# dotchen/LAV

Hardware: NVIDIA H100
Metric: agent_frames_per_s (higher is better)
Workload: dtype fp16 storage, fp32 accumulate (wgmma f16 / mma.sync f16; saturating stores)

## Files before the change

### include/lav_b200.h

```cpp
#ifndef LAV_B200_H
#define LAV_B200_H

#include <stddef.h>
#include <stdint.h>

#ifdef __cplusplus
extern "C" {
#endif

#define LAVB_ABI_VERSION 3

int lavb_abi_version(void);
const char* lavb_last_error(void);
int lavb_device_cc(void);

enum { LAVB_F32 = 0, LAVB_BF16 = 1, LAVB_F16 = 2 };
int lavb_h16_dtype(void);

int lavb_paint(const float* d_pts, int n, int pt_stride,
               const float* d_sem, int ncam, int c_in, int h, int w,
               long long s_cam, long long s_c, long long s_y, long long s_x,
               const float* h_cams, int mode,
               float* d_out, int out_stride, int out_col0, int copy_cols, void* stream);

// ... 180 lines not shown
size_t lavb_det_peaks_workspace_bytes(int batch, int ncls);
int lavb_det_peaks(const float* d_center, const float* d_box, const float* d_ori, int batch, int h, int w, int ncls,
                   float min_score, int max_det, float* d_packed, void* d_workspace, void* stream);

int lavb_crop_bilinear(const void* d_feat, int dtype, int b, int h, int w, int c, const int* d_frame_idx,
                       const float* d_theta, int k, int crop, void* d_out, void* stream);
int lavb_crop_bilinear_u8(const uint8_t* d_map, int b, int c, int h, int w, const int* d_frame_idx, const float* d_theta,
                          int k, int crop, float* d_out, void* stream);
int lavb_crop_bilinear_bwd(const float* d_gout, int b, int h, int w, int c, const int* d_frame_idx, const float* d_theta,
                           int k, int crop, float* d_gfeat, void* stream);

int lavb_convert(const void* d_src, int src_dtype, void* d_dst, int dst_dtype, long long count, void* stream);

int lavb_conv_umma(const lavb_conv_desc* h_desc, void* stream);

int lavb_conv7x7s2_umma(const void* d_in, int n, int h, int w, int cin, const void* d_w, const float* d_bias, void* d_out,
                        void* stream);

int lavb_conv3x3_umma(const void* d_in, int n, int h, int w, int cin, int stride, const void* d_w, int cout, const float* d_bias,
                      const float* d_scale, const float* d_shift, int pre_relu, void* d_out, void* stream);

typedef struct lavb_conv_pair_desc {
  const void* in; void* out; const void* res;
  int n, h, w, c, dil, post_relu;
  const void* w1; const float* bias1;
  const void* w2; const float* shift2;
} lavb_conv_pair_desc;
int lavb_conv_pair_umma(const lavb_conv_pair_desc* h_desc, void* stream);
int lavb_conv_pair_set_trace(void* d_buf, int tiles_per_cta);

// ... 15 lines not shown
```

### lav_b200/capi.py

```python
import ctypes as C
import os

_HERE = os.path.dirname(os.path.abspath(__file__))
LIB_PATH = os.path.join(_HERE, "_lib", "liblavb200.so")

F32, BF16, F16 = 0, 1, 2


class LavbError(RuntimeError):
    pass


class ConvDesc(C.Structure):
    _fields_ = [
        ("inp", C.c_void_p), ("in_dtype", C.c_int), ("n", C.c_int), ("hin", C.c_int), ("win", C.c_int), ("cin", C.c_int),
        ("in_cstride", C.c_int), ("in_coff", C.c_int),
        ("out", C.c_void_p), ("out_dtype", C.c_int), ("hout", C.c_int), ("wout", C.c_int), ("cout", C.c_int),
        ("out_cstride", C.c_int), ("out_coff", C.c_int),
        ("hog", C.c_int), ("wog", C.c_int),
        ("in_sy", C.c_int), ("in_sx", C.c_int), ("out_sy", C.c_int), ("out_sx", C.c_int), ("out_oy", C.c_int), ("out_ox", C.c_int),
        ("ntaps", C.c_int), ("dy", C.c_int * 16), ("dx", C.c_int * 16),
        ("w", C.c_void_p), ("bias", C.c_void_p), ("scale", C.c_void_p), ("shift", C.c_void_p),
        ("res", C.c_void_p), ("res_dtype", C.c_int), ("res_cstride", C.c_int), ("res_coff", C.c_int),
        ("pre_relu", C.c_int), ("post_relu", C.c_int), ("sigmoid", C.c_int), ("d2s_nout", C.c_int),
    ]


class ConvPairDesc(C.Structure):
    _fields_ = [
        ("inp", C.c_void_p), ("out", C.c_void_p), ("res", C.c_void_p),
        ("n", C.c_int), ("h", C.c_int), ("w", C.c_int), ("c", C.c_int), ("dil", C.c_int), ("post_relu", C.c_int),
        ("w1", C.c_void_p), ("bias1", C.c_void_p),
        ("w2", C.c_void_p), ("shift2", C.c_void_p),
    ]


class ControlConfig(C.Structure):
    _fields_ = [
        ("aim_point", C.c_int * 8), ("speed_ratio", C.c_double * 8),
# ... 103 lines not shown
    "lavb_det_peaks_workspace_bytes": (C.c_size_t, [C.c_int, C.c_int]),
    "lavb_det_peaks": (C.c_int, [C.c_void_p, C.c_void_p, C.c_void_p, C.c_int, C.c_int, C.c_int, C.c_int, C.c_float, C.c_int,
                                 C.c_void_p, C.c_void_p, C.c_void_p]),
    "lavb_crop_bilinear": (C.c_int, [C.c_void_p, C.c_int, C.c_int, C.c_int, C.c_int, C.c_int, C.c_void_p, C.c_void_p, C.c_int,
                                     C.c_int, C.c_void_p, C.c_void_p]),
    "lavb_crop_bilinear_u8": (C.c_int, [C.c_void_p, C.c_int, C.c_int, C.c_int, C.c_int, C.c_void_p, C.c_void_p, C.c_int, C.c_int,
                                        C.c_void_p, C.c_void_p]),
    "lavb_cast_gru": (C.c_int, [C.c_void_p, C.c_int, C.c_void_p, C.c_void_p, C.c_void_p, C.c_void_p, C.c_void_p, C.c_void_p, C.c_int,
                                C.c_int, C.c_void_p, C.c_void_p]),
    "lavb_conv_pair_set_trace": (C.c_int, [C.c_void_p, C.c_int]),
    "lavb_crop_bilinear_bwd": (C.c_int, [C.c_void_p, C.c_int, C.c_int, C.c_int, C.c_int, C.c_void_p, C.c_void_p, C.c_int, C.c_int,
                                         C.c_void_p, C.c_void_p]),
    "lavb_deconv3x3s2_small": (C.c_int, [C.c_void_p, C.c_int, C.c_int, C.c_int, C.c_int, C.c_int, C.c_int, C.c_int, C.c_void_p,
                                         C.c_void_p, C.c_void_p, C.c_void_p, C.c_void_p, C.c_void_p]),
    "lavb_conv_umma": (C.c_int, [C.POINTER(ConvDesc), C.c_void_p]),
    "lavb_conv7x7s2_umma": (C.c_int, [C.c_void_p, C.c_int, C.c_int, C.c_int, C.c_int, C.c_void_p, C.c_void_p, C.c_void_p,
                                      C.c_void_p]),
    "lavb_conv3x3_umma": (C.c_int, [C.c_void_p, C.c_int, C.c_int, C.c_int, C.c_int, C.c_int, C.c_void_p, C.c_int, C.c_void_p,
                                    C.c_void_p, C.c_void_p, C.c_int, C.c_void_p, C.c_void_p]),
}

_lib = None


def exported_symbols():
    return sorted(_SIGS)


def lib():
    global _lib
# ... 23 lines not shown
```

### lav_b200/csrc/conv_umma.cu

```cuda
#include "sm90.cuh"

namespace lavb {

constexpr int kTileH = 8, kTileW = 16, kBlockM = 128, kBlockK = 64;
constexpr int kABytes = kBlockM * kBlockK * 2;
constexpr int kMaxStages = 8;
constexpr int kMaxTaps = 16;
constexpr int kConvThreads = 288;

struct ConvArgs {
  int n, hog, wog, tiles_x, tiles_y, num_tiles;
  int hout, wout, cin, cout, kchunks, ntaps, stages;
  int in_sy, in_sx, out_sy, out_sx, out_oy, out_ox;
  int out_cstride, out_coff, out_is_f32, res_cstride, res_coff;
  int pre_bias, pre_relu, post_relu, sigmoid, d2s_nout, cout_store;
  int dy[kMaxTaps], dx[kMaxTaps];
  void* out; const h16* res;
  const float* bias; const float* scale; const float* shift;
};

using namespace sm90;

template <int kNC>
__global__ void __launch_bounds__(kConvThreads, kNC <= 4 ? 2 : 1) conv_umma_kernel(const __grid_constant__ CUtensorMap tmap_a,
                                                                                 const __grid_constant__ CUtensorMap tmap_b,
                                                                                 const __grid_constant__ ConvArgs p) {
  constexpr int kN = 32 * kNC;
  constexpr int kBBytes = kN * kBlockK * 2;
  constexpr int kStageBytes = kABytes + kBBytes;
  extern __shared__ uint8_t smem_raw[];
  const uint32_t base = (smem_u32(smem_raw) + 1023u) & ~1023u;
  uint8_t* gen = smem_raw + (base - smem_u32(smem_raw));
  const uint32_t ctrl = base + p.stages * kStageBytes;
  const uint32_t full_bar = ctrl, empty_bar = ctrl + 8 * kMaxStages;
  float* ep_bias = reinterpret_cast<float*>(gen + (ctrl - base) + 16 * kMaxStages);
  float* ep_st = ep_bias + 256;

  const int warp = threadIdx.x >> 5, lane = threadIdx.x & 31;
  if (threadIdx.x == 0) {
    asm volatile("prefetch.tensormap [%0];" ::"l"(reinterpret_cast<uint64_t>(&tmap_a)) : "memory");
    asm volatile("prefetch.tensormap [%0];" ::"l"(reinterpret_cast<uint64_t>(&tmap_b)) : "memory");
    for (int s = 0; s < p.stages; ++s) { mbar_init(full_bar + 8 * s, 1); mbar_init(empty_bar + 8 * s, 8); }
    asm volatile("fence.mbarrier_init.release.cluster;" ::: "memory");
  }
  for (int c = threadIdx.x; c < kN; c += blockDim.x) {
    const bool real = c < p.cout_store;
    const float b = (p.bias && real) ? __ldg(p.bias + c) : 0.f;
    const float sc = (p.scale && real) ? __ldg(p.scale + c) : 1.f;
    const float sh = (p.shift && real) ? __ldg(p.shift + c) : 0.f;
    ep_bias[c] = b;
    ep_st[2 * c] = sc;
    ep_st[2 * c + 1] = p.pre_bias ? sh : fmaf(b, sc, sh);
  }
  __syncthreads();
  const int nkb = p.ntaps * p.kchunks;
  const int tiles_per_img = p.tiles_x * p.tiles_y;

  if (warp == 8) {
    if (lane == 0) {
      int stage = 0; uint32_t phase = 0;
      for (int tile = blockIdx.x; tile < p.num_tiles; tile += gridDim.x) {
        const int img = tile / tiles_per_img, r = tile - img * tiles_per_img;
        const int y0 = (r / p.tiles_x) * kTileH * p.in_sy, x0 = (r % p.tiles_x) * kTileW * p.in_sx;
        for (int t = 0; t < p.ntaps; ++t) {
          for (int kc = 0; kc < p.kchunks; ++kc) {
            mbar_wait(empty_bar + 8 * stage, phase ^ 1);
            const uint32_t sa = base + stage * kStageBytes;
            mbar_expect_tx(full_bar + 8 * stage, kStageBytes);
            tma_load_4d(sa, &tmap_a, full_bar + 8 * stage, kc * kBlockK, x0 + p.dx[t], y0 + p.dy[t], img);
            tma_load_2d(sa + kABytes, &tmap_b, full_bar + 8 * stage, kc * kBlockK, t * kN);
            if (++stage == p.stages) { stage = 0; phase ^= 1; }
          }
        }
      }
    }
    return;
  }

  const int wg = warp >> 2;
  const float lo_pre = p.pre_relu ? 0.f : -INFINITY, lo_post = p.post_relu ? 0.f : -INFINITY;
  int stage = 0; uint32_t phase = 0;
  float acc[16 * kNC];
  for (int tile = blockIdx.x; tile < p.num_tiles; tile += gridDim.x) {
    int prev_stage = -1;
    for (int kb = 0; kb < nkb; ++kb) {
      mbar_wait(full_bar + 8 * stage, phase);
      const uint32_t sa = base + stage * kStageBytes;
      const uint64_t a_desc = sm90::desc_sw128(sa + wg * (kABytes / 2)), b_desc = sm90::desc_sw128(sa + kABytes);
      sm90::wgmma_fence();
#pragma unroll
      for (int k = 0; k < kBlockK / 16; ++k)
        sm90::wgmma<kN>(acc, a_desc + (uint64_t)(2 * k), b_desc + (uint64_t)(2 * k), (kb | k) ? 1u : 0u);
      sm90::wgmma_commit();
      sm90::wgmma_wait<1>();
      if (prev_stage >= 0 && lane == 0) mbar_arrive(empty_bar + 8 * prev_stage);
      prev_stage = stage;
      if (++stage == p.stages) { stage = 0; phase ^= 1; }
    }
    sm90::wgmma_wait<0>();
    sm90::acc_fence(acc);
    if (prev_stage >= 0 && lane == 0) mbar_arrive(empty_bar + 8 * prev_stage);

    const int c0 = 2 * (lane & 3), store_lim = p.cout_store - c0;
    const int img = tile / tiles_per_img, r = tile - img * tiles_per_img;
    const int gy = (r / p.tiles_x) * kTileH + 4 * wg + (warp & 3), oy = gy * p.out_sy + p.out_oy;
    if (!(gy < p.hog && oy < p.hout)) continue;
#pragma unroll
    for (int h = 0; h < 2; ++h) {
      const int gx = (r % p.tiles_x) * kTileW + (lane >> 2) + 8 * h, ox = gx * p.out_sx + p.out_ox;
      if (!(gx < p.wog && ox < p.wout)) continue;
      const long long pix = ((long long)img * p.hout + oy) * p.wout + ox;
      uint8_t* out_at = reinterpret_cast<uint8_t*>(p.out) + (pix * p.out_cstride + p.out_coff + c0) * (p.out_is_f32 ? 4 : 2);
      const h16* res_at = p.res ? p.res + pix * p.res_cstride + p.res_coff + c0 : nullptr;
      const float* bias_at = ep_bias + c0;
      const float* st_at = ep_st + 2 * c0;
#pragma unroll
      for (int j = 0; j < 4 * kNC; ++j) {
        const int g = 8 * j;
        float x0 = acc[4 * j + 2 * h], x1 = acc[4 * j + 2 * h + 1];
        if (p.pre_bias) { x0 += bias_at[g]; x1 += bias_at[g + 1]; }
        const float4 st = *reinterpret_cast<const float4*>(st_at + 2 * g);
        x0 = fmaf(fmaxf(x0, lo_pre), st.x, st.y);
        x1 = fmaf(fmaxf(x1, lo_pre), st.z, st.w);
        if (res_at) {
          const float2 rv = unpack_h16(__ldg(reinterpret_cast<const uint32_t*>(res_at + g)));
          x0 += rv.x; x1 += rv.y;
        }
        x0 = fmaxf(x0, lo_post); x1 = fmaxf(x1, lo_post);
        if (p.sigmoid) { x0 = 1.f / (1.f + expf(-x0)); x1 = 1.f / (1.f + expf(-x1)); }
        if (kNC == 1 && p.d2s_nout) {
          float* ob = reinterpret_cast<float*>(p.out);
          const int no = p.d2s_nout;
#pragma unroll
          for (int e = 0; e < 2; ++e) {
            const int q = g + c0 + e;
            if (q < 4 * no) {
              const int pos = q / no, k = q - pos * no;
              ob[(pix + (long long)(pos >> 1) * p.wout + (pos & 1)) * no + k] = e ? x1 : x0;
            }
          }
        } else if (g < store_lim) {
          if (p.out_is_f32)
            *reinterpret_cast<float2*>(out_at + 4 * g) = make_float2(x0, x1);
          else
            *reinterpret_cast<uint32_t*>(out_at + 2 * g) = pack_h16(x0, x1);
        }
      }
    }
  }
}

}

using namespace lavb;

extern "C" int lavb_conv_umma(const lavb_conv_desc* d, void* stream) {
  LAVB_CHECK_ARG(d != nullptr, "conv_umma: null descriptor");
  LAVB_CHECK_ARG(d->in_dtype == LAVB_H16, "conv_umma: input must be h16");
  LAVB_CHECK_ARG(d->out_dtype == LAVB_H16 || d->out_dtype == LAVB_F32, "conv_umma: bad output dtype");
  LAVB_CHECK_ARG(d->ntaps >= 1 && d->ntaps <= kMaxTaps, "conv_umma: ntaps must be 1..16");
  LAVB_CHECK_ARG(d->cin % 64 == 0 && d->cin > 0, "conv_umma: cin must be a multiple of 64 (got %d)", d->cin);
  LAVB_CHECK_ARG(d->cout % 8 == 0 && d->cout >= 8 && d->cout <= 256, "conv_umma: cout must be 8..256, multiple of 8 (got %d)", d->cout);
  const int cout_mma = (d->cout + 31) / 32 * 32;
  LAVB_CHECK_ARG(d->res == nullptr || cout_mma == d->cout, "conv_umma: residual needs cout %% 32 == 0");
  LAVB_CHECK_ARG(d->in_cstride % 8 == 0 && d->in_coff % 8 == 0 && d->in_coff + d->cin <= d->in_cstride, "conv_umma: input slice misaligned");
  LAVB_CHECK_ARG(d->out_cstride % 8 == 0 && d->out_coff % 8 == 0 && d->out_coff + d->cout <= d->out_cstride, "conv_umma: output slice misaligned");
  LAVB_CHECK_ARG(d->res == nullptr || (d->res_dtype == LAVB_H16 && d->res_cstride % 8 == 0 && d->res_coff % 8 == 0), "conv_umma: residual must be h16, 16 B aligned");
  LAVB_CHECK_ARG((d->scale == nullptr) == (d->shift == nullptr), "conv_umma: scale and shift come together");
  LAVB_CHECK_ARG(d->in_sy >= 1 && d->in_sy <= 8 && d->in_sx >= 1 && d->in_sx <= 8, "conv_umma: bad input stride");
  auto encode = get_encode();
  LAVB_CHECK_ARG(encode != nullptr, "conv_umma: cuTensorMapEncodeTiled not available from the driver");

  CUtensorMap tmap_a, tmap_b;
  {
    const h16* in = reinterpret_cast<const h16*>(d->in) + d->in_coff;
    cuuint64_t dims[4] = {(cuuint64_t)d->cin, (cuuint64_t)d->win, (cuuint64_t)d->hin, (cuuint64_t)d->n};
    cuuint64_t strides[3] = {(cuuint64_t)d->in_cstride * 2, (cuuint64_t)d->win * d->in_cstride * 2,
                             (cuuint64_t)d->hin * d->win * d->in_cstride * 2};
    cuuint32_t box[4] = {(cuuint32_t)kBlockK, (cuuint32_t)(kTileW * d->in_sx), (cuuint32_t)(kTileH * d->in_sy), 1};
    cuuint32_t estr[4] = {1, (cuuint32_t)d->in_sx, (cuuint32_t)d->in_sy, 1};
    CUresult r = encode(&tmap_a, LAVB_TMAP_H16, 4, const_cast<h16*>(in), dims, strides, box, estr,
                        CU_TENSOR_MAP_INTERLEAVE_NONE, CU_TENSOR_MAP_SWIZZLE_128B, CU_TENSOR_MAP_L2_PROMOTION_L2_256B,
                        CU_TENSOR_MAP_FLOAT_OOB_FILL_NONE);
    LAVB_CHECK_ARG(r == CUDA_SUCCESS, "conv_umma: cuTensorMapEncodeTiled(A) failed with %d", (int)r);
  }
  {
    cuuint64_t dims[2] = {(cuuint64_t)d->cin, (cuuint64_t)d->ntaps * cout_mma};
    cuuint64_t strides[1] = {(cuuint64_t)d->cin * 2};
    cuuint32_t box[2] = {(cuuint32_t)kBlockK, (cuuint32_t)cout_mma};
    cuuint32_t estr[2] = {1, 1};
    CUresult r = encode(&tmap_b, LAVB_TMAP_H16, 2, const_cast<float*>(d->w), dims, strides, box, estr,
                        CU_TENSOR_MAP_INTERLEAVE_NONE, CU_TENSOR_MAP_SWIZZLE_128B, CU_TENSOR_MAP_L2_PROMOTION_L2_256B,
                        CU_TENSOR_MAP_FLOAT_OOB_FILL_NONE);
    LAVB_CHECK_ARG(r == CUDA_SUCCESS, "conv_umma: cuTensorMapEncodeTiled(B) failed with %d", (int)r);
  }
  ConvArgs a;
  memset(&a, 0, sizeof(a));
  a.n = d->n; a.hog = d->hog; a.wog = d->wog;
  a.tiles_x = ceil_div(d->wog, kTileW); a.tiles_y = ceil_div(d->hog, kTileH);
  a.num_tiles = a.n * a.tiles_x * a.tiles_y;
  a.hout = d->hout; a.wout = d->wout; a.cin = d->cin; a.cout = cout_mma; a.cout_store = d->cout; a.kchunks = d->cin / kBlockK;
  a.ntaps = d->ntaps;
  const int nc = cout_mma / 32;
  const bool two_per_sm = nc <= 4;
  const int stage_bytes = kABytes + cout_mma * kBlockK * 2;
  const int ctrl_bytes = 1024  + 16 * kMaxStages + 3 * 256 * (int)sizeof(float);
  const int smem_cap = two_per_sm ? 113 * 1024 : 227 * 1024;
  a.stages = min(kMaxStages, (smem_cap - ctrl_bytes) / stage_bytes);
  a.in_sy = d->in_sy; a.in_sx = d->in_sx; a.out_sy = d->out_sy; a.out_sx = d->out_sx; a.out_oy = d->out_oy; a.out_ox = d->out_ox;
  a.out_cstride = d->out_cstride; a.out_coff = d->out_coff; a.out_is_f32 = d->out_dtype == LAVB_F32;
  a.res_cstride = d->res_cstride; a.res_coff = d->res_coff;
  a.pre_bias = d->pre_relu && d->bias != nullptr;
  a.pre_relu = d->pre_relu; a.post_relu = d->post_relu; a.sigmoid = d->sigmoid; a.d2s_nout = d->d2s_nout;
  if (d->d2s_nout) {
    LAVB_CHECK_ARG(d->cout == 32 && d->d2s_nout >= 1 && 4 * d->d2s_nout <= 32 && d->out_dtype == LAVB_F32 && d->out_sy == 2 &&
                   d->out_sx == 2 && d->res == nullptr, "conv_umma: depth-to-space epilogue needs cout=32, fp32 out, out_s=2, no residual");
  }
  for (int t = 0; t < d->ntaps; ++t) { a.dy[t] = d->dy[t]; a.dx[t] = d->dx[t]; }
  a.out = d->out; a.res = reinterpret_cast<const h16*>(d->res);
  a.bias = d->bias; a.scale = d->scale; a.shift = d->shift;
  if (a.num_tiles == 0) return 0;
  const int smem = a.stages * stage_bytes + ctrl_bytes;
  const int grid = min(a.num_tiles, two_per_sm ? 2 * kNumSMs : kNumSMs);
#define LAVB_CONV_LAUNCH(NC)                                                                                              \
  case NC: {                                                                                                              \
                             \
    LAVB_CUDA_OK(ensure_dyn_smem((const void*)conv_umma_kernel<NC>, smem_cap));                                          \
    conv_umma_kernel<NC><<<grid, kConvThreads, smem, (cudaStream_t)stream>>>(tmap_a, tmap_b, a);                          \
    break;                                                                                                                \
  }
  switch (nc) {
    LAVB_CONV_LAUNCH(1) LAVB_CONV_LAUNCH(2) LAVB_CONV_LAUNCH(3) LAVB_CONV_LAUNCH(4)
    LAVB_CONV_LAUNCH(5) LAVB_CONV_LAUNCH(6) LAVB_CONV_LAUNCH(7) LAVB_CONV_LAUNCH(8)
  }
#undef LAVB_CONV_LAUNCH
  LAVB_LAUNCH_OK();
  return 0;
}
```

### lav_b200/layers.py

```python
import torch

from . import ops

USE_UMMA = True
UMMA_STRIDED = True


def bn_affine(bn, eps=None):
    eps = bn.eps if eps is None else eps
    var = bn.running_var.double()
    scale = bn.weight.double() / torch.sqrt(var + eps)
    shift = bn.bias.double() - bn.running_mean.double() * scale
    return scale.float().contiguous(), shift.float().contiguous()


def _pad_cout(w_tco):
    t, ci, co = w_tco.shape
    cp = (co + 15) // 16 * 16
    out = torch.zeros((t, ci, cp), dtype=torch.float32, device=w_tco.device)
    out[:, :, :co] = w_tco
    return out.contiguous()


def cmajor_wins(hout, wout):
# ... 39 lines not shown
                                continue
                            taps.append(((oy + py_ - ky * dy_) // sy, (ox + px_ - kx * dx_) // sx))
                            blocks.append(self._block(w[:, :, ky, kx]))
                    if not taps:
                        taps, blocks = [(0, 0)], [torch.zeros((self.cin_k, self.cout), device=w.device)]
                    self.phases.append(dict(taps=taps, w=_pad_cout(torch.stack(blocks)), in_s=(1, 1), out_s=(sy, sx),
                                            out_o=(oy, ox)))
        for ph in self.phases:
            assert len(ph["taps"]) <= 16, "tap list longer than the kernel's table"
        self.umma_ok = USE_UMMA and self.cin_k % 64 == 0 and self.cout % 8 == 0 and self.cout <= 256
        self.cmajor_ok = (self.umma_ok and not transposed and (self.kh, self.kw) == (3, 3) and self.padding == (1, 1)
                          and self.dilation == (1, 1) and self.stride in ((1, 1), (2, 2)) and self.cin_k in (64, 128, 384)
                          and self.cout in (64, 128, 256) and not post_relu and not sigmoid)
        if self.umma_ok:
            cm = (self.cout + 31) // 32 * 32
            for ph in self.phases:
                wu = torch.zeros((len(ph["taps"]), cm, self.cin_k), dtype=ops.h16(), device=ph["w"].device)
                wu[:, :self.cout] = ph["w"][:, :, :self.cout].permute(0, 2, 1).to(ops.h16())
                ph["w_umma"] = wu.contiguous()

    def _block(self, w_ci_co):
        if self.cin_k == self.cin:
            return w_ci_co
        out = torch.zeros((self.cin_k, self.cout), dtype=w_ci_co.dtype, device=w_ci_co.device)
        out[:self.cin] = w_ci_co
        return out

    def out_size(self, hin, win):
        (sy, sx), (py_, px_), (dy_, dx_), (oy, ox) = self.stride, self.padding, self.dilation, self.opad
        if self.transposed:
            return ((hin - 1) * sy - 2 * py_ + dy_ * (self.kh - 1) + oy + 1, (win - 1) * sx - 2 * px_ + dx_ * (self.kw - 1) + ox + 1)
        return ((hin + 2 * py_ - dy_ * (self.kh - 1) - 1) // sy + 1, (win + 2 * px_ - dx_ * (self.kw - 1) - 1) // sx + 1)

    def __call__(self, x, out=None, in_coff=0, out_coff=0, out_channels=None, res=None, res_coff=0, out_dtype=None):
        n, hin, win, _ = x.shape
        hout, wout = self.out_size(hin, win)
        if out is None:
            out = torch.empty((n, hout, wout, out_channels or self.cout), dtype=out_dtype or x.dtype, device=x.device)
        if (self.cmajor_ok and cmajor_wins(hout, wout) and x.dtype == ops.h16()
                and out.dtype == ops.h16() and x.shape[3] == self.cin_k and in_coff == 0 and out.shape[3] == self.cout
                and out_coff == 0 and res is None):
            ph = self.phases[0]
            return ops.conv3x3_umma(x, ph["w_umma"], self.cout, self.stride[0], self.bias, self.scale, self.shift, self.pre_relu,
                                    out=out)
        for ph in self.phases:
            osy, osx = ph["out_s"]
            ooy, oox = ph["out_o"]
            hog, wog = (hout - ooy + osy - 1) // osy, (wout - oox + osx - 1) // osx
            umma = (self.umma_ok and x.dtype == ops.h16() and (res is None or (res.dtype == ops.h16() and self.cout % 32 == 0))
                    and (UMMA_STRIDED or ph["in_s"] == (1, 1)))
            ops.conv_taps(x, self.cin_k, in_coff, out, self.cout, out_coff, hog, wog, ph["in_s"], ph["out_s"], ph["out_o"],
                          ph["taps"], ph["w_umma"] if umma else ph["w"], self.bias, self.scale, self.shift, res, res_coff,
                          self.pre_relu, self.post_relu, self.sigmoid, umma=umma)
        return out


class PlanMixin:

    def _plan_get(self, device, builder):
        plans = self.__dict__.setdefault("_lavb_plans", {})
        key = (str(device), getattr(self, "precision", "fp32"))
        if key not in plans:
            with torch.no_grad():
                plans[key] = builder(device)
        return plans[key]
# ... 18 lines not shown
```

### lav_b200/lidar.py

```python
import torch
from torch import nn

from . import ops
from .capi import LavbError
from .layers import PlanMixin, TapConv, bn_affine
from .point_pillar import PointPillarNet


def _dt(precision):
    return torch.float32 if precision == "fp32" else ops.h16()


def _nhwc(x):
    if not x.is_cuda:
        raise LavbError("lav_b200 modules need CUDA tensors (no CPU fallback)")
    return x.permute(0, 2, 3, 1).contiguous()


class ConvBackbone(PlanMixin, nn.Module):
    def __init__(self, num_feature=64, norm_cfg={'eps': 1e-3, 'momentum': 0.01}):
        super().__init__()
        nf = num_feature

        def stage(cin, cout, n):
# ... 141 lines not shown
            no = ct.out_channels
            wd[g, :, :, :no] = ct.weight.detach().float().permute(0, 2, 3, 1).reshape(nh, 9, no)
            bd[g, :no] = ct.bias.detach().float()
            n_outs.append(no)
            w = ct.weight.detach().float()
            wu = torch.zeros((4, 32, nh), dtype=torch.float32, device=device)
            opts = {0: [(0, 1)], 1: [(0, 2), (1, 0)]}
            for pa in (0, 1):
                for pb in (0, 1):
                    for dy, ky in opts[pa]:
                        for dx, kx in opts[pb]:
                            wu[dy * 2 + dx, (pa * 2 + pb) * no:(pa * 2 + pb) * no + no] = w[:, :, ky, kx].t()
            bias32 = torch.zeros(32, dtype=torch.float32, device=device)
            bias32[:4 * no] = ct.bias.detach().float().repeat(4)
            d2s.append((wu.to(ops.h16()).contiguous(), bias32))
        return conv, (wd.contiguous(), bd.contiguous(), n_outs, [h._is_sigmoid() for h in self._heads()], nh, d2s)

    def heads_nhwc(self, feats):
        conv, (wd, bd, n_outs, sig, nh, d2s) = self._plan_get(feats.device, self._build)
        if self.precision == "f16":
            hid = conv(feats, out_dtype=ops.h16())
            n, h, w, _ = hid.shape
            outs = []
            for g, (wu, b32) in enumerate(d2s):
                out = torch.empty((n, 2 * h, 2 * w, n_outs[g]), dtype=torch.float32, device=hid.device)
                ops.conv_taps(hid, nh, g * nh, out, 32, 0, h, w, (1, 1), (2, 2), (0, 0), [(0, 0), (0, 1), (1, 0), (1, 1)], wu,
                              bias=b32, sigmoid=sig[g], umma=True, d2s_nout=n_outs[g])
                outs.append(out)
            return outs
        hid = conv(feats, out_dtype=torch.float32)
        return ops.deconv3x3s2_small(hid, 4, nh, wd, bd, n_outs, sig)

    def forward_nhwc(self, lidars, num_points):
        canvas = self.point_pillar_net.forward_nhwc(lidars, num_points, canvas16=self.precision == "f16")
        feats = self.backbone.forward_nhwc(canvas)
        return (feats, *self.heads_nhwc(feats))

    def forward(self, lidars, num_points):
        if self.training:
            from .train import lidar_model_train_forward
            return lidar_model_train_forward(self, lidars, num_points)
        return tuple(t.permute(0, 3, 1, 2) for t in self.forward_nhwc(lidars, num_points))
```

### lav_b200/ops.py

```python
import ctypes as C
import math

import numpy as np
import torch

from . import capi
from .capi import BF16, F16, F32, ConvDesc, check, lib

_DT = {torch.float32: F32, torch.bfloat16: BF16, torch.float16: F16}


def h16():
    return torch.float16 if capi.h16_code() == F16 else torch.bfloat16



def _stream():
    return C.c_void_p(torch.cuda.current_stream().cuda_stream)


def _ptr(t):
    return C.c_void_p(t.data_ptr()) if t is not None else C.c_void_p(0)


# ... 194 lines not shown
        d.dy[i], d.dx[i] = dy, dx
    d.w = w.data_ptr()
    d.bias = bias.data_ptr() if bias is not None else None
    d.scale = scale.data_ptr() if scale is not None else None
    d.shift = shift.data_ptr() if shift is not None else None
    if res is not None:
        assert res.is_contiguous() and res.shape[:3] == out.shape[:3]
        d.res, d.res_dtype, d.res_cstride, d.res_coff = res.data_ptr(), _DT[res.dtype], res.shape[3], res_coff
    d.pre_relu, d.post_relu, d.sigmoid = int(pre_relu), int(post_relu), int(sigmoid)
    if umma:
        e0 = _prof_begin()
        check(lib().lavb_conv_umma(C.byref(d), _stream()), "lavb_conv_umma")
        _prof_end(f"umma:{cin}->{cout}x{len(taps)}taps@{hog}x{wog}", 2.0 * x.shape[0] * hog * wog * cout * cin * len(taps), e0)
    else:
        check(lib().lavb_conv_taps(C.byref(d), _stream()), "lavb_conv_taps")
    _COUNT[0] += 1
    return out


def pool2_affine_relu(x, c, in_coff, scale, shift, out, out_coff):
    _need_cuda(x, out)
    n, h, w, cs = x.shape
    check(lib().lavb_pool2_affine_relu(_ptr(x), _DT[x.dtype], n, h, w, c, cs, in_coff, _ptr(scale), _ptr(shift), _ptr(out),
                                       out.shape[3], out_coff, _stream()), "lavb_pool2_affine_relu")
    _COUNT[0] += 1
    return out


def rgb_normalize(rgb, out_dtype=torch.float32):
    _need_cuda(rgb)
# ... 1047 lines not shown
```

Baseline: 2067.

## Merge multi-phase tap convolutions and detection heads into one UMMA launch

Adds a phase-table variant of the UMMA conv kernel so that all sub-pixel phases of a strided or transposed TapConv, and all depth-to-space detection heads, run in a single persistent launch instead of one launch per phase or head. Tiles from the different phases are interleaved across CTAs, and per-phase geometry, tap offsets, input channel offsets, outputs and biases are read from a table staged in shared memory. This is meant to cut launch count and tail underutilisation on small grids. In exchange it adds per-tile table lookups, more shared memory, and a larger kernel argument block.

```diff
diff --git a/include/lav_b200.h b/include/lav_b200.h
--- a/include/lav_b200.h
+++ b/include/lav_b200.h
@@ -218,6 +218,14 @@
 
 int lavb_conv_umma(const lavb_conv_desc* h_desc, void* stream);
 
+typedef struct {
+  int hog, wog, out_oy, out_ox;
+  int ntaps, tap0; int dy[16]; int dx[16];
+  int in_coff;
+  void* out; const float* bias; int sigmoid, d2s_nout;
+} lavb_conv_phase;
+int lavb_conv_umma_phases(const lavb_conv_desc* h_desc, const lavb_conv_phase* h_phases, int nphases, void* stream);
+
 int lavb_conv7x7s2_umma(const void* d_in, int n, int h, int w, int cin, const void* d_w, const float* d_bias, void* d_out,
                         void* stream);
 
diff --git a/lav_b200/capi.py b/lav_b200/capi.py
--- a/lav_b200/capi.py
+++ b/lav_b200/capi.py
@@ -23,6 +23,15 @@
         ("w", C.c_void_p), ("bias", C.c_void_p), ("scale", C.c_void_p), ("shift", C.c_void_p),
         ("res", C.c_void_p), ("res_dtype", C.c_int), ("res_cstride", C.c_int), ("res_coff", C.c_int),
         ("pre_relu", C.c_int), ("post_relu", C.c_int), ("sigmoid", C.c_int), ("d2s_nout", C.c_int),
+    ]
+
+
+class ConvPhase(C.Structure):
+    _fields_ = [
+        ("hog", C.c_int), ("wog", C.c_int), ("out_oy", C.c_int), ("out_ox", C.c_int),
+        ("ntaps", C.c_int), ("tap0", C.c_int), ("dy", C.c_int * 16), ("dx", C.c_int * 16),
+        ("in_coff", C.c_int),
+        ("out", C.c_void_p), ("bias", C.c_void_p), ("sigmoid", C.c_int), ("d2s_nout", C.c_int),
     ]
 
 
@@ -156,6 +165,7 @@
     "lavb_deconv3x3s2_small": (C.c_int, [C.c_void_p, C.c_int, C.c_int, C.c_int, C.c_int, C.c_int, C.c_int, C.c_int, C.c_void_p,
                                          C.c_void_p, C.c_void_p, C.c_void_p, C.c_void_p, C.c_void_p]),
     "lavb_conv_umma": (C.c_int, [C.POINTER(ConvDesc), C.c_void_p]),
+    "lavb_conv_umma_phases": (C.c_int, [C.POINTER(ConvDesc), C.POINTER(ConvPhase), C.c_int, C.c_void_p]),
     "lavb_conv7x7s2_umma": (C.c_int, [C.c_void_p, C.c_int, C.c_int, C.c_int, C.c_int, C.c_void_p, C.c_void_p, C.c_void_p,
                                       C.c_void_p]),
     "lavb_conv3x3_umma": (C.c_int, [C.c_void_p, C.c_int, C.c_int, C.c_int, C.c_int, C.c_int, C.c_void_p, C.c_int, C.c_void_p,
diff --git a/lav_b200/csrc/conv_umma.cu b/lav_b200/csrc/conv_umma.cu
--- a/lav_b200/csrc/conv_umma.cu
+++ b/lav_b200/csrc/conv_umma.cu
@@ -6,25 +6,50 @@
 constexpr int kABytes = kBlockM * kBlockK * 2;
 constexpr int kMaxStages = 8;
 constexpr int kMaxTaps = 16;
+constexpr int kMaxSubs = 16;
+constexpr int kMaxTapRows = 64;
 constexpr int kConvThreads = 288;
 
-struct ConvArgs {
-  int n, hog, wog, tiles_x, tiles_y, num_tiles;
-  int hout, wout, cin, cout, kchunks, ntaps, stages;
-  int in_sy, in_sx, out_sy, out_sx, out_oy, out_ox;
+struct ConvSub {
+  int tile0, tiles_x, tiles_per_img;
+  int hog, wog, out_oy, out_ox;
+  int ntaps, tap0, in_coff;
+  int ep_col, flags;
+  void* out;
+};
+
+struct ConvHead {
+  int num_tiles, nsub, nep, ntap_rows, interleave;
+  int hout, wout, cout, kchunks, stages;
+  int in_sy, in_sx, out_sy, out_sx;
   int out_cstride, out_coff, out_is_f32, res_cstride, res_coff;
-  int pre_bias, pre_relu, post_relu, sigmoid, d2s_nout, cout_store;
-  int dy[kMaxTaps], dx[kMaxTaps];
-  void* out; const h16* res;
-  const float* bias; const float* scale; const float* shift;
+  int pre_relu, post_relu, cout_store;
+  const h16* res; const float* scale; const float* shift;
 };
 
+template <int kSubs>
+struct ConvArgs : ConvHead {
+  int dy[kSubs == 1 ? kMaxTaps : kMaxTapRows], dx[kSubs == 1 ? kMaxTaps : kMaxTapRows];
+  ConvSub sub[kSubs];
+  const float* bias[kSubs];
+};
+
 using namespace sm90;
 
-template <int kNC>
+constexpr int kTableBytes = kMaxSubs * (int)sizeof(ConvSub) + 2 * kMaxTapRows * (int)sizeof(int);
+
+__device__ __forceinline__ int locate(const ConvSub* subs, int nsub, int interleave, int tile, int s, int& r) {
+  if (interleave) { r = tile / nsub; return tile - r * nsub; }
+  while (s + 1 < nsub && tile >= subs[s + 1].tile0) ++s;
+  r = tile - subs[s].tile0;
+  return s;
+}
+
+template <int kNC, int kSubs>
 __global__ void __launch_bounds__(kConvThreads, kNC <= 4 ? 2 : 1) conv_umma_kernel(const __grid_constant__ CUtensorMap tmap_a,
                                                                                  const __grid_constant__ CUtensorMap tmap_b,
-                                                                                 const __grid_constant__ ConvArgs p) {
+                                                                                 const __grid_constant__ ConvArgs<kSubs> p) {
+  constexpr bool kTable = kSubs > 1;
   constexpr int kN = 32 * kNC;
   constexpr int kBBytes = kN * kBlockK * 2;
   constexpr int kStageBytes = kABytes + kBBytes;
@@ -35,6 +60,19 @@
   const uint32_t full_bar = ctrl, empty_bar = ctrl + 8 * kMaxStages;
   float* ep_bias = reinterpret_cast<float*>(gen + (ctrl - base) + 16 * kMaxStages);
   float* ep_st = ep_bias + 256;
+  ConvSub* subs = reinterpret_cast<ConvSub*>(ep_st + 512);
+  int* tap_dy = reinterpret_cast<int*>(subs + kMaxSubs);
+  int* tap_dx = tap_dy + kMaxTapRows;
+  auto sub = [&](int s) -> const ConvSub& {
+    if constexpr (kTable) return subs[s]; else return p.sub[0];
+  };
+  auto tap_y = [&](int t) { if constexpr (kTable) return tap_dy[t]; else return p.dy[t]; };
+  auto tap_x = [&](int t) { if constexpr (kTable) return tap_dx[t]; else return p.dx[t]; };
+  auto find = [&](int tile, int s, int& r) {
+    if constexpr (kTable) return locate(subs, p.nsub, p.interleave, tile, s, r);
+    r = tile;
+    return 0;
+  };
 
   const int warp = threadIdx.x >> 5, lane = threadIdx.x & 31;
   if (threadIdx.x == 0) {
@@ -43,31 +81,40 @@
     for (int s = 0; s < p.stages; ++s) { mbar_init(full_bar + 8 * s, 1); mbar_init(empty_bar + 8 * s, 8); }
     asm volatile("fence.mbarrier_init.release.cluster;" ::: "memory");
   }
-  for (int c = threadIdx.x; c < kN; c += blockDim.x) {
+  for (int i = threadIdx.x; i < p.nep * kN; i += blockDim.x) {
+    const int e = i / kN, c = i - e * kN;
     const bool real = c < p.cout_store;
-    const float b = (p.bias && real) ? __ldg(p.bias + c) : 0.f;
+    const float* bias = p.bias[e];
+    const float b = (bias && real) ? __ldg(bias + c) : 0.f;
     const float sc = (p.scale && real) ? __ldg(p.scale + c) : 1.f;
     const float sh = (p.shift && real) ? __ldg(p.shift + c) : 0.f;
-    ep_bias[c] = b;
-    ep_st[2 * c] = sc;
-    ep_st[2 * c + 1] = p.pre_bias ? sh : fmaf(b, sc, sh);
+    ep_bias[i] = b;
+    ep_st[2 * i] = sc;
+    ep_st[2 * i + 1] = (p.pre_relu && bias) ? sh : fmaf(b, sc, sh);
+  }
+  if constexpr (kTable) {
+    for (int i = threadIdx.x; i < p.nsub * (int)(sizeof(ConvSub) / 4); i += blockDim.x)
+      reinterpret_cast<int*>(subs)[i] = reinterpret_cast<const int*>(p.sub)[i];
+    for (int i = threadIdx.x; i < p.ntap_rows; i += blockDim.x) { tap_dy[i] = p.dy[i]; tap_dx[i] = p.dx[i]; }
   }
   __syncthreads();
-  const int nkb = p.ntaps * p.kchunks;
-  const int tiles_per_img = p.tiles_x * p.tiles_y;
 
   if (warp == 8) {
     if (lane == 0) {
-      int stage = 0; uint32_t phase = 0;
+      int stage = 0, s = 0; uint32_t phase = 0;
       for (int tile = blockIdx.x; tile < p.num_tiles; tile += gridDim.x) {
-        const int img = tile / tiles_per_img, r = tile - img * tiles_per_img;
-        const int y0 = (r / p.tiles_x) * kTileH * p.in_sy, x0 = (r % p.tiles_x) * kTileW * p.in_sx;
-        for (int t = 0; t < p.ntaps; ++t) {
+        int r;
+        s = find(tile, s, r);
+        const ConvSub& sb = sub(s);
+        const int img = r / sb.tiles_per_img;
+        r -= img * sb.tiles_per_img;
+        const int y0 = (r / sb.tiles_x) * kTileH * p.in_sy, x0 = (r % sb.tiles_x) * kTileW * p.in_sx;
+        for (int t = sb.tap0; t < sb.tap0 + sb.ntaps; ++t) {
           for (int kc = 0; kc < p.kchunks; ++kc) {
             mbar_wait(empty_bar + 8 * stage, phase ^ 1);
             const uint32_t sa = base + stage * kStageBytes;
             mbar_expect_tx(full_bar + 8 * stage, kStageBytes);
-            tma_load_4d(sa, &tmap_a, full_bar + 8 * stage, kc * kBlockK, x0 + p.dx[t], y0 + p.dy[t], img);
+            tma_load_4d(sa, &tmap_a, full_bar + 8 * stage, sb.in_coff + kc * kBlockK, x0 + tap_x(t), y0 + tap_y(t), img);
             tma_load_2d(sa + kABytes, &tmap_b, full_bar + 8 * stage, kc * kBlockK, t * kN);
             if (++stage == p.stages) { stage = 0; phase ^= 1; }
           }
@@ -79,9 +126,12 @@
 
   const int wg = warp >> 2;
   const float lo_pre = p.pre_relu ? 0.f : -INFINITY, lo_post = p.post_relu ? 0.f : -INFINITY;
-  int stage = 0; uint32_t phase = 0;
+  int stage = 0, si = 0; uint32_t phase = 0;
   float acc[16 * kNC];
   for (int tile = blockIdx.x; tile < p.num_tiles; tile += gridDim.x) {
+    int r;
+    si = find(tile, si, r);
+    const int nkb = sub(si).ntaps * p.kchunks;
     int prev_stage = -1;
     for (int kb = 0; kb < nkb; ++kb) {
       mbar_wait(full_bar + 8 * stage, phase);
@@ -102,23 +152,29 @@
     if (prev_stage >= 0 && lane == 0) mbar_arrive(empty_bar + 8 * prev_stage);
 
     const int c0 = 2 * (lane & 3), store_lim = p.cout_store - c0;
-    const int img = tile / tiles_per_img, r = tile - img * tiles_per_img;
-    const int gy = (r / p.tiles_x) * kTileH + 4 * wg + (warp & 3), oy = gy * p.out_sy + p.out_oy;
-    if (!(gy < p.hog && oy < p.hout)) continue;
+    int sj = si;
+    const int img = r / sub(sj).tiles_per_img;
+    r -= img * sub(sj).tiles_per_img;
+    const int gy = (r / sub(sj).tiles_x) * kTileH + 4 * wg + (warp & 3), oy = gy * p.out_sy + sub(sj).out_oy;
+    if (!(gy < sub(sj).hog && oy < p.hout)) continue;
+    int gx0 = (r % sub(sj).tiles_x) * kTileW + (lane >> 2), pix_row = img * p.hout + oy;
 #pragma unroll
     for (int h = 0; h < 2; ++h) {
-      const int gx = (r % p.tiles_x) * kTileW + (lane >> 2) + 8 * h, ox = gx * p.out_sx + p.out_ox;
-      if (!(gx < p.wog && ox < p.wout)) continue;
-      const long long pix = ((long long)img * p.hout + oy) * p.wout + ox;
-      uint8_t* out_at = reinterpret_cast<uint8_t*>(p.out) + (pix * p.out_cstride + p.out_coff + c0) * (p.out_is_f32 ? 4 : 2);
+      asm volatile("" : "+r"(sj), "+r"(gx0), "+r"(pix_row));
+      const ConvSub& sb = sub(sj);
+      const int flags = sb.flags;
+      const float* bias_at = ep_bias + sb.ep_col + c0;
+      const float* st_at = ep_st + 2 * (sb.ep_col + c0);
+      const int gx = gx0 + 8 * h, ox = gx * p.out_sx + sb.out_ox;
+      if (!(gx < sb.wog && ox < p.wout)) continue;
+      const long long pix = (long long)pix_row * p.wout + ox;
+      uint8_t* out_at = reinterpret_cast<uint8_t*>(sb.out) + (pix * p.out_cstride + p.out_coff + c0) * (p.out_is_f32 ? 4 : 2);
       const h16* res_at = p.res ? p.res + pix * p.res_cstride + p.res_coff + c0 : nullptr;
-      const float* bias_at = ep_bias + c0;
-      const float* st_at = ep_st + 2 * c0;
 #pragma unroll
       for (int j = 0; j < 4 * kNC; ++j) {
         const int g = 8 * j;
         float x0 = acc[4 * j + 2 * h], x1 = acc[4 * j + 2 * h + 1];
-        if (p.pre_bias) { x0 += bias_at[g]; x1 += bias_at[g + 1]; }
+        if (flags & 1) { x0 += bias_at[g]; x1 += bias_at[g + 1]; }
         const float4 st = *reinterpret_cast<const float4*>(st_at + 2 * g);
         x0 = fmaf(fmaxf(x0, lo_pre), st.x, st.y);
         x1 = fmaf(fmaxf(x1, lo_pre), st.z, st.w);
@@ -127,10 +183,10 @@
           x0 += rv.x; x1 += rv.y;
         }
         x0 = fmaxf(x0, lo_post); x1 = fmaxf(x1, lo_post);
-        if (p.sigmoid) { x0 = 1.f / (1.f + expf(-x0)); x1 = 1.f / (1.f + expf(-x1)); }
-        if (kNC == 1 && p.d2s_nout) {
-          float* ob = reinterpret_cast<float*>(p.out);
-          const int no = p.d2s_nout;
+        if (flags & 2) { x0 = 1.f / (1.f + expf(-x0)); x1 = 1.f / (1.f + expf(-x1)); }
+        if (kNC == 1 && (flags >> 2)) {
+          float* ob = reinterpret_cast<float*>(sb.out);
+          const int no = flags >> 2;
 #pragma unroll
           for (int e = 0; e < 2; ++e) {
             const int q = g + c0 + e;
@@ -154,27 +210,51 @@
 
 using namespace lavb;
 
-extern "C" int lavb_conv_umma(const lavb_conv_desc* d, void* stream) {
-  LAVB_CHECK_ARG(d != nullptr, "conv_umma: null descriptor");
+namespace {
+
+int conv_umma_launch(const lavb_conv_desc* d, const lavb_conv_phase* ph, int nph, void* stream) {
+  LAVB_CHECK_ARG(d != nullptr && ph != nullptr, "conv_umma: null descriptor or table");
+  LAVB_CHECK_ARG(nph >= 1 && nph <= kMaxSubs, "conv_umma: the table must have 1..16 entries (got %d)", nph);
   LAVB_CHECK_ARG(d->in_dtype == LAVB_H16, "conv_umma: input must be h16");
   LAVB_CHECK_ARG(d->out_dtype == LAVB_H16 || d->out_dtype == LAVB_F32, "conv_umma: bad output dtype");
-  LAVB_CHECK_ARG(d->ntaps >= 1 && d->ntaps <= kMaxTaps, "conv_umma: ntaps must be 1..16");
+  LAVB_CHECK_ARG(d->ntaps >= 1 && d->ntaps <= kMaxTapRows, "conv_umma: the weight tensor must hold 1..64 taps (got %d)", d->ntaps);
   LAVB_CHECK_ARG(d->cin % 64 == 0 && d->cin > 0, "conv_umma: cin must be a multiple of 64 (got %d)", d->cin);
   LAVB_CHECK_ARG(d->cout % 8 == 0 && d->cout >= 8 && d->cout <= 256, "conv_umma: cout must be 8..256, multiple of 8 (got %d)", d->cout);
   const int cout_mma = (d->cout + 31) / 32 * 32;
   LAVB_CHECK_ARG(d->res == nullptr || cout_mma == d->cout, "conv_umma: residual needs cout %% 32 == 0");
-  LAVB_CHECK_ARG(d->in_cstride % 8 == 0 && d->in_coff % 8 == 0 && d->in_coff + d->cin <= d->in_cstride, "conv_umma: input slice misaligned");
+  LAVB_CHECK_ARG(d->in_cstride % 8 == 0, "conv_umma: input slice misaligned");
   LAVB_CHECK_ARG(d->out_cstride % 8 == 0 && d->out_coff % 8 == 0 && d->out_coff + d->cout <= d->out_cstride, "conv_umma: output slice misaligned");
   LAVB_CHECK_ARG(d->res == nullptr || (d->res_dtype == LAVB_H16 && d->res_cstride % 8 == 0 && d->res_coff % 8 == 0), "conv_umma: residual must be h16, 16 B aligned");
   LAVB_CHECK_ARG((d->scale == nullptr) == (d->shift == nullptr), "conv_umma: scale and shift come together");
   LAVB_CHECK_ARG(d->in_sy >= 1 && d->in_sy <= 8 && d->in_sx >= 1 && d->in_sx <= 8, "conv_umma: bad input stride");
+  int coff_lo = d->in_cstride, coff_hi = 0, nep = 0;
+  const float* eps[kMaxSubs];
+  for (int i = 0; i < nph; ++i) {
+    const lavb_conv_phase& e = ph[i];
+    LAVB_CHECK_ARG(e.ntaps >= 1 && e.ntaps <= kMaxTaps, "conv_umma: entry %d: ntaps must be 1..16", i);
+    LAVB_CHECK_ARG(e.tap0 >= 0 && e.tap0 + e.ntaps <= d->ntaps, "conv_umma: entry %d: taps [%d, %d) outside the weight tensor's %d",
+                   i, e.tap0, e.tap0 + e.ntaps, d->ntaps);
+    LAVB_CHECK_ARG(e.in_coff >= 0 && e.in_coff % 8 == 0 && e.in_coff + d->cin <= d->in_cstride, "conv_umma: entry %d: input slice misaligned", i);
+    LAVB_CHECK_ARG(e.hog >= 0 && e.wog >= 0 && e.out_oy >= 0 && e.out_ox >= 0, "conv_umma: entry %d: negative output grid or origin", i);
+    LAVB_CHECK_ARG(e.out != nullptr, "conv_umma: entry %d: null output", i);
+    if (e.d2s_nout) {
+      LAVB_CHECK_ARG(d->cout == 32 && e.d2s_nout >= 1 && 4 * e.d2s_nout <= 32 && d->out_dtype == LAVB_F32 && d->out_sy == 2 &&
+                     d->out_sx == 2 && d->res == nullptr, "conv_umma: depth-to-space epilogue needs cout=32, fp32 out, out_s=2, no residual");
+    }
+    coff_lo = min(coff_lo, e.in_coff);
+    coff_hi = max(coff_hi, e.in_coff);
+    int k = 0;
+    while (k < nep && eps[k] != e.bias) ++k;
+    if (k == nep) eps[nep++] = e.bias;
+  }
+  LAVB_CHECK_ARG(nep * cout_mma <= 256, "conv_umma: %d distinct biases of %d columns exceed 256 epilogue columns", nep, cout_mma);
   auto encode = get_encode();
   LAVB_CHECK_ARG(encode != nullptr, "conv_umma: cuTensorMapEncodeTiled not available from the driver");
 
   CUtensorMap tmap_a, tmap_b;
   {
-    const h16* in = reinterpret_cast<const h16*>(d->in) + d->in_coff;
-    cuuint64_t dims[4] = {(cuuint64_t)d->cin, (cuuint64_t)d->win, (cuuint64_t)d->hin, (cuuint64_t)d->n};
+    const h16* in = reinterpret_cast<const h16*>(d->in) + coff_lo;
+    cuuint64_t dims[4] = {(cuuint64_t)(coff_hi - coff_lo + d->cin), (cuuint64_t)d->win, (cuuint64_t)d->hin, (cuuint64_t)d->n};
     cuuint64_t strides[3] = {(cuuint64_t)d->in_cstride * 2, (cuuint64_t)d->win * d->in_cstride * 2,
                              (cuuint64_t)d->hin * d->win * d->in_cstride * 2};
     cuuint32_t box[4] = {(cuuint32_t)kBlockK, (cuuint32_t)(kTileW * d->in_sx), (cuuint32_t)(kTileH * d->in_sy), 1};
@@ -194,39 +274,66 @@
                         CU_TENSOR_MAP_FLOAT_OOB_FILL_NONE);
     LAVB_CHECK_ARG(r == CUDA_SUCCESS, "conv_umma: cuTensorMapEncodeTiled(B) failed with %d", (int)r);
   }
-  ConvArgs a;
+  ConvArgs<kMaxSubs> a;
   memset(&a, 0, sizeof(a));
-  a.n = d->n; a.hog = d->hog; a.wog = d->wog;
-  a.tiles_x = ceil_div(d->wog, kTileW); a.tiles_y = ceil_div(d->hog, kTileH);
-  a.num_tiles = a.n * a.tiles_x * a.tiles_y;
-  a.hout = d->hout; a.wout = d->wout; a.cin = d->cin; a.cout = cout_mma; a.cout_store = d->cout; a.kchunks = d->cin / kBlockK;
-  a.ntaps = d->ntaps;
+  a.nsub = nph; a.nep = nep; a.ntap_rows = d->ntaps;
+  a.interleave = 1;
+  long long tiles = 0;
+  for (int i = 0; i < nph; ++i) {
+    const lavb_conv_phase& e = ph[i];
+    ConvSub& s = a.sub[i];
+    s.tile0 = (int)tiles;
+    s.tiles_x = ceil_div(e.wog, kTileW);
+    s.tiles_per_img = s.tiles_x * ceil_div(e.hog, kTileH);
+    tiles += (long long)d->n * s.tiles_per_img;
+    s.hog = e.hog; s.wog = e.wog; s.out_oy = e.out_oy; s.out_ox = e.out_ox;
+    s.ntaps = e.ntaps; s.tap0 = e.tap0; s.in_coff = e.in_coff - coff_lo;
+    int ep = 0;
+    while (eps[ep] != e.bias) ++ep;
+    s.ep_col = ep * cout_mma;
+    s.flags = (d->pre_relu && e.bias != nullptr) | (e.sigmoid ? 2 : 0) | e.d2s_nout << 2;
+    a.interleave &= s.tiles_per_img == a.sub[0].tiles_per_img && s.ntaps == a.sub[0].ntaps && s.flags == a.sub[0].flags;
+    s.out = e.out;
+    for (int t = 0; t < e.ntaps; ++t) { a.dy[e.tap0 + t] = e.dy[t]; a.dx[e.tap0 + t] = e.dx[t]; }
+  }
+  LAVB_CHECK_ARG(tiles < (1ll << 31), "conv_umma: %lld tiles exceed the int tile index", tiles);
+  for (int i = 0; i < nph; ++i)
+    for (int t = 0; t < ph[i].ntaps; ++t)
+      LAVB_CHECK_ARG(a.dy[ph[i].tap0 + t] == ph[i].dy[t] && a.dx[ph[i].tap0 + t] == ph[i].dx[t],
+                     "conv_umma: entry %d: weight tap %d is given two different offsets", i, ph[i].tap0 + t);
+  a.num_tiles = (int)tiles;
+  a.hout = d->hout; a.wout = d->wout; a.cout = cout_mma; a.cout_store = d->cout; a.kchunks = d->cin / kBlockK;
   const int nc = cout_mma / 32;
   const bool two_per_sm = nc <= 4;
   const int stage_bytes = kABytes + cout_mma * kBlockK * 2;
-  const int ctrl_bytes = 1024  + 16 * kMaxStages + 3 * 256 * (int)sizeof(float);
+  const int ctrl_bytes = 1024  + 16 * kMaxStages + 3 * 256 * (int)sizeof(float) + (nph > 1 ? kTableBytes : 0);
   const int smem_cap = two_per_sm ? 113 * 1024 : 227 * 1024;
   a.stages = min(kMaxStages, (smem_cap - ctrl_bytes) / stage_bytes);
-  a.in_sy = d->in_sy; a.in_sx = d->in_sx; a.out_sy = d->out_sy; a.out_sx = d->out_sx; a.out_oy = d->out_oy; a.out_ox = d->out_ox;
+  a.in_sy = d->in_sy; a.in_sx = d->in_sx; a.out_sy = d->out_sy; a.out_sx = d->out_sx;
   a.out_cstride = d->out_cstride; a.out_coff = d->out_coff; a.out_is_f32 = d->out_dtype == LAVB_F32;
   a.res_cstride = d->res_cstride; a.res_coff = d->res_coff;
-  a.pre_bias = d->pre_relu && d->bias != nullptr;
-  a.pre_relu = d->pre_relu; a.post_relu = d->post_relu; a.sigmoid = d->sigmoid; a.d2s_nout = d->d2s_nout;
-  if (d->d2s_nout) {
-    LAVB_CHECK_ARG(d->cout == 32 && d->d2s_nout >= 1 && 4 * d->d2s_nout <= 32 && d->out_dtype == LAVB_F32 && d->out_sy == 2 &&
-                   d->out_sx == 2 && d->res == nullptr, "conv_umma: depth-to-space epilogue needs cout=32, fp32 out, out_s=2, no residual");
-  }
-  for (int t = 0; t < d->ntaps; ++t) { a.dy[t] = d->dy[t]; a.dx[t] = d->dx[t]; }
-  a.out = d->out; a.res = reinterpret_cast<const h16*>(d->res);
-  a.bias = d->bias; a.scale = d->scale; a.shift = d->shift;
+  for (int k = 0; k < nep; ++k) a.bias[k] = eps[k];
+  a.pre_relu = d->pre_relu; a.post_relu = d->post_relu;
+  a.res = reinterpret_cast<const h16*>(d->res);
+  a.scale = d->scale; a.shift = d->shift;
   if (a.num_tiles == 0) return 0;
   const int smem = a.stages * stage_bytes + ctrl_bytes;
   const int grid = min(a.num_tiles, two_per_sm ? 2 * kNumSMs : kNumSMs);
+  ConvArgs<1> a1;
+  memset(&a1, 0, sizeof(a1));
+  static_cast<ConvHead&>(a1) = a;
+  for (int t = 0; t < kMaxTaps; ++t) { a1.dy[t] = a.dy[t]; a1.dx[t] = a.dx[t]; }
+  a1.sub[0] = a.sub[0]; a1.bias[0] = a.bias[0];
 #define LAVB_CONV_LAUNCH(NC)                                                                                              \
   case NC: {                                                                                                              \
                              \
-    LAVB_CUDA_OK(ensure_dyn_smem((const void*)conv_umma_kernel<NC>, smem_cap));                                          \
-    conv_umma_kernel<NC><<<grid, kConvThreads, smem, (cudaStream_t)stream>>>(tmap_a, tmap_b, a);                          \
+    if (nph == 1) {                                                                                                       \
+      LAVB_CUDA_OK(ensure_dyn_smem((const void*)conv_umma_kernel<NC, 1>, smem_cap));                                     \
+      conv_umma_kernel<NC, 1><<<grid, kConvThreads, smem, (cudaStream_t)stream>>>(tmap_a, tmap_b, a1);                   \
+    } else {                                                                                                              \
+      LAVB_CUDA_OK(ensure_dyn_smem((const void*)conv_umma_kernel<NC, kMaxSubs>, smem_cap));                              \
+      conv_umma_kernel<NC, kMaxSubs><<<grid, kConvThreads, smem, (cudaStream_t)stream>>>(tmap_a, tmap_b, a);             \
+    }                                                                                                                     \
     break;                                                                                                                \
   }
   switch (nc) {
@@ -237,3 +344,21 @@
   LAVB_LAUNCH_OK();
   return 0;
 }
+
+}
+
+extern "C" int lavb_conv_umma(const lavb_conv_desc* d, void* stream) {
+  LAVB_CHECK_ARG(d != nullptr, "conv_umma: null descriptor");
+  LAVB_CHECK_ARG(d->ntaps >= 1 && d->ntaps <= kMaxTaps, "conv_umma: ntaps must be 1..16");
+  lavb_conv_phase e;
+  memset(&e, 0, sizeof(e));
+  e.hog = d->hog; e.wog = d->wog; e.out_oy = d->out_oy; e.out_ox = d->out_ox;
+  e.ntaps = d->ntaps; e.tap0 = 0;
+  for (int t = 0; t < d->ntaps; ++t) { e.dy[t] = d->dy[t]; e.dx[t] = d->dx[t]; }
+  e.in_coff = d->in_coff; e.out = d->out; e.bias = d->bias; e.sigmoid = d->sigmoid; e.d2s_nout = d->d2s_nout;
+  return conv_umma_launch(d, &e, 1, stream);
+}
+
+extern "C" int lavb_conv_umma_phases(const lavb_conv_desc* d, const lavb_conv_phase* h_phases, int nphases, void* stream) {
+  return conv_umma_launch(d, h_phases, nphases, stream);
+}
diff --git a/lav_b200/layers.py b/lav_b200/layers.py
--- a/lav_b200/layers.py
+++ b/lav_b200/layers.py
@@ -4,6 +4,7 @@
 
 USE_UMMA = True
 UMMA_STRIDED = True
+UMMA_ONE_LAUNCH = True
 
 
 def bn_affine(bn, eps=None):
@@ -77,10 +78,15 @@
                           and self.cout in (64, 128, 256) and not post_relu and not sigmoid)
         if self.umma_ok:
             cm = (self.cout + 31) // 32 * 32
+            w_all = torch.zeros((sum(len(ph["taps"]) for ph in self.phases), cm, self.cin_k), dtype=ops.h16(),
+                                device=self.phases[0]["w"].device)
+            t0 = 0
             for ph in self.phases:
-                wu = torch.zeros((len(ph["taps"]), cm, self.cin_k), dtype=ops.h16(), device=ph["w"].device)
-                wu[:, :self.cout] = ph["w"][:, :, :self.cout].permute(0, 2, 1).to(ops.h16())
-                ph["w_umma"] = wu.contiguous()
+                nt = len(ph["taps"])
+                w_all[t0:t0 + nt, :self.cout] = ph["w"][:, :, :self.cout].permute(0, 2, 1).to(ops.h16())
+                ph["w_umma"], ph["tap0"] = w_all[t0:t0 + nt], t0
+                t0 += nt
+            self.w_umma = w_all
 
     def _block(self, w_ci_co):
         if self.cin_k == self.cin:
@@ -106,12 +112,18 @@
             ph = self.phases[0]
             return ops.conv3x3_umma(x, ph["w_umma"], self.cout, self.stride[0], self.bias, self.scale, self.shift, self.pre_relu,
                                     out=out)
+        grid = lambda ph: ((hout - ph["out_o"][0] + ph["out_s"][0] - 1) // ph["out_s"][0],
+                           (wout - ph["out_o"][1] + ph["out_s"][1] - 1) // ph["out_s"][1])
+        umma = (self.umma_ok and x.dtype == ops.h16() and (res is None or (res.dtype == ops.h16() and self.cout % 32 == 0))
+                and (UMMA_STRIDED or self.phases[0]["in_s"] == (1, 1)))
+        if umma and UMMA_ONE_LAUNCH and 1 < len(self.phases) <= 16 and self.w_umma.shape[0] <= 64:
+            ph0 = self.phases[0]
+            table = [dict(hog=grid(ph)[0], wog=grid(ph)[1], out_o=ph["out_o"], taps=ph["taps"], tap0=ph["tap0"], in_coff=in_coff,
+                          bias=self.bias, sigmoid=self.sigmoid) for ph in self.phases]
+            return ops.conv_umma_phases(x, self.cin_k, out, self.cout, out_coff, ph0["in_s"], ph0["out_s"], self.w_umma, table,
+                                        self.scale, self.shift, res, res_coff, self.pre_relu, self.post_relu)
         for ph in self.phases:
-            osy, osx = ph["out_s"]
-            ooy, oox = ph["out_o"]
-            hog, wog = (hout - ooy + osy - 1) // osy, (wout - oox + osx - 1) // osx
-            umma = (self.umma_ok and x.dtype == ops.h16() and (res is None or (res.dtype == ops.h16() and self.cout % 32 == 0))
-                    and (UMMA_STRIDED or ph["in_s"] == (1, 1)))
+            hog, wog = grid(ph)
             ops.conv_taps(x, self.cin_k, in_coff, out, self.cout, out_coff, hog, wog, ph["in_s"], ph["out_s"], ph["out_o"],
                           ph["taps"], ph["w_umma"] if umma else ph["w"], self.bias, self.scale, self.shift, res, res_coff,
                           self.pre_relu, self.post_relu, self.sigmoid, umma=umma)
diff --git a/lav_b200/lidar.py b/lav_b200/lidar.py
--- a/lav_b200/lidar.py
+++ b/lav_b200/lidar.py
@@ -1,7 +1,7 @@
 import torch
 from torch import nn
 
-from . import ops
+from . import layers, ops
 from .capi import LavbError
 from .layers import PlanMixin, TapConv, bn_affine
 from .point_pillar import PointPillarNet
@@ -179,19 +179,24 @@
             bias32 = torch.zeros(32, dtype=torch.float32, device=device)
             bias32[:4 * no] = ct.bias.detach().float().repeat(4)
             d2s.append((wu.to(ops.h16()).contiguous(), bias32))
-        return conv, (wd.contiguous(), bd.contiguous(), n_outs, [h._is_sigmoid() for h in self._heads()], nh, d2s)
+        w_d2s = torch.cat([wu for wu, _ in d2s]).contiguous()
+        return conv, (wd.contiguous(), bd.contiguous(), n_outs, [h._is_sigmoid() for h in self._heads()], nh, d2s, w_d2s)
 
     def heads_nhwc(self, feats):
-        conv, (wd, bd, n_outs, sig, nh, d2s) = self._plan_get(feats.device, self._build)
+        conv, (wd, bd, n_outs, sig, nh, d2s, w_d2s) = self._plan_get(feats.device, self._build)
         if self.precision == "f16":
             hid = conv(feats, out_dtype=ops.h16())
             n, h, w, _ = hid.shape
-            outs = []
-            for g, (wu, b32) in enumerate(d2s):
-                out = torch.empty((n, 2 * h, 2 * w, n_outs[g]), dtype=torch.float32, device=hid.device)
-                ops.conv_taps(hid, nh, g * nh, out, 32, 0, h, w, (1, 1), (2, 2), (0, 0), [(0, 0), (0, 1), (1, 0), (1, 1)], wu,
-                              bias=b32, sigmoid=sig[g], umma=True, d2s_nout=n_outs[g])
-                outs.append(out)
+            outs = [torch.empty((n, 2 * h, 2 * w, no), dtype=torch.float32, device=hid.device) for no in n_outs]
+            taps = [(0, 0), (0, 1), (1, 0), (1, 1)]
+            if not layers.UMMA_ONE_LAUNCH:
+                for g, (wu, b32) in enumerate(d2s):
+                    ops.conv_taps(hid, nh, g * nh, outs[g], 32, 0, h, w, (1, 1), (2, 2), (0, 0), taps, wu, bias=b32,
+                                  sigmoid=sig[g], umma=True, d2s_nout=n_outs[g])
+                return outs
+            table = [dict(hog=h, wog=w, out_o=(0, 0), taps=taps, tap0=4 * g, in_coff=g * nh, out=outs[g], bias=b32,
+                          sigmoid=sig[g], d2s_nout=n_outs[g]) for g, (_, b32) in enumerate(d2s)]
+            ops.conv_umma_phases(hid, nh, outs[0], 32, 0, (1, 1), (2, 2), w_d2s, table)
             return outs
         hid = conv(feats, out_dtype=torch.float32)
         return ops.deconv3x3s2_small(hid, 4, nh, wd, bd, n_outs, sig)
diff --git a/lav_b200/ops.py b/lav_b200/ops.py
--- a/lav_b200/ops.py
+++ b/lav_b200/ops.py
@@ -232,6 +232,56 @@
         _prof_end(f"umma:{cin}->{cout}x{len(taps)}taps@{hog}x{wog}", 2.0 * x.shape[0] * hog * wog * cout * cin * len(taps), e0)
     else:
         check(lib().lavb_conv_taps(C.byref(d), _stream()), "lavb_conv_taps")
+    _COUNT[0] += 1
+    return out
+
+
+def conv_umma_phases(x, cin, out, cout, out_coff, in_s, out_s, w, phases, scale=None, shift=None, res=None, res_coff=0,
+                     pre_relu=False, post_relu=False):
+    _need_cuda(x, out, w)
+    assert x.is_contiguous() and out.is_contiguous() and w.is_contiguous() and x.dtype == h16() and w.dtype == h16()
+    assert w.dim() == 3 and w.shape[1:] == ((cout + 31) // 32 * 32, cin) and 1 <= len(phases) <= 16
+    d = ConvDesc()
+    d.inp, d.in_dtype = x.data_ptr(), _DT[x.dtype]
+    d.n, d.hin, d.win, d.in_cstride = x.shape
+    d.cin = cin
+    d.out, d.out_dtype = out.data_ptr(), _DT[out.dtype]
+    assert out.shape[0] == x.shape[0]
+    _, d.hout, d.wout, d.out_cstride = out.shape
+    d.cout, d.out_coff = cout, out_coff
+    d.in_sy, d.in_sx = in_s
+    d.out_sy, d.out_sx = out_s
+    d.ntaps = w.shape[0]
+    d.w = w.data_ptr()
+    d.scale = scale.data_ptr() if scale is not None else None
+    d.shift = shift.data_ptr() if shift is not None else None
+    if res is not None:
+        assert res.is_contiguous() and res.shape[:3] == out.shape[:3]
+        d.res, d.res_dtype, d.res_cstride, d.res_coff = res.data_ptr(), _DT[res.dtype], res.shape[3], res_coff
+    d.pre_relu, d.post_relu = int(pre_relu), int(post_relu)
+    table = (capi.ConvPhase * len(phases))()
+    fl = 0.0
+    for e, ph in zip(table, phases):
+        o = ph.get("out", out)
+        e.hog, e.wog = ph["hog"], ph["wog"]
+        e.out_oy, e.out_ox = ph["out_o"]
+        e.ntaps, e.tap0 = len(ph["taps"]), ph["tap0"]
+        for i, (dy, dx) in enumerate(ph["taps"]):
+            e.dy[i], e.dx[i] = dy, dx
+        e.in_coff = ph.get("in_coff", 0)
+        e.d2s_nout = ph.get("d2s_nout", 0)
+        if e.d2s_nout:
+            assert o.dtype == torch.float32 and o.shape[3] == e.d2s_nout and cout == 32 and 4 * e.d2s_nout <= 32
+            d.out_cstride, d.out_coff = 32, 0
+        assert o.is_contiguous() and o.device == out.device and o.dtype == out.dtype and o.shape[:3] == out.shape[:3]
+        e.out = o.data_ptr()
+        bias = ph.get("bias")
+        e.bias = bias.data_ptr() if bias is not None else None
+        e.sigmoid = int(ph.get("sigmoid", False))
+        fl += 2.0 * x.shape[0] * e.hog * e.wog * cout * cin * e.ntaps
+    e0 = _prof_begin()
+    check(lib().lavb_conv_umma_phases(C.byref(d), table, len(phases), _stream()), "lavb_conv_umma_phases")
+    _prof_end(f"umma:{cin}->{cout}x{len(phases)}phases@{phases[0]['hog']}x{phases[0]['wog']}", fl, e0)
     _COUNT[0] += 1
     return out
 
```

Result: no change. 2069, median of 6 (+0.1%).
